# NilFoundation/crypto3-fil-proofs

Hardware: AMD Instinct MI355X
Metric: Groth16 constraints/sec (BLS12-381); MSM G1 Mpoints/s at 2^26 (higher is better)
Workload: dtype u32 limbs (Fq 381-bit / Fr 255-bit Montgomery)

## Files before the change

crypto3-fil-proofs_amd/csrc/ctx.h:

```cpp
#pragma once
#include <hip/hip_runtime.h>
#include <stdint.h>

#include <atomic>
#include <mutex>
#include <stdexcept>
#include <string>
#include <vector>

#include "curve.h"
#include "field.h"
#include "fr29.h"
#include "tune.h"

namespace mi {

struct hip_error : std::runtime_error {
    hipError_t code;
    hip_error(hipError_t c, const std::string &what) : std::runtime_error(what), code(c) {}
};

#define MI_HIP(call)                                                                              \
    do {                                                                                          \
        hipError_t _e = (call);                                                                   \
// ... 139 lines not shown
                keep.push_back(p);
                continue;
            }
            float ms = 0;
            hipEventElapsedTime(&ms, p.a, p.b);
            p.dst->ms += ms;
            p.dst->launches += 1;
            p.dst->units += p.units;
            pool.push_back(p.a);
            pool.push_back(p.b);
        }
        pending.swap(keep);
    }
    ~EventTimer() {
        for (auto &p : pending) {
            hipEventDestroy(p.a);
            hipEventDestroy(p.b);
        }
        for (auto e : pool) hipEventDestroy(e);
    }
};

inline uint64_t next_ctx_uid() {
    static std::atomic<uint64_t> n{1};
    return n.fetch_add(1);
}

struct Ctx {
    const uint64_t uid = next_ctx_uid();
    int device = 0;
    hipStream_t stream = nullptr;
    std::recursive_mutex mu;
    NttTables tw;
    DevBuf scratch[34];
    Stats stats;
    EventTimer timer;
    PinnedBuf pin;
    int64_t inject_oom = 0;
    Ctx *aux = nullptr;
    hipStream_t aux_streams[2] = {nullptr, nullptr};
    hipStream_t plan_stream = nullptr;
    hipEvent_t plan_ev[2] = {nullptr, nullptr};
};

Ctx &ctx_aux(Ctx &c);
void ctx_aux_free(Ctx &c);

struct ScopedTimer {
    Ctx &c;
    KStat *dst;
    uint64_t units;
    hipEvent_t a;
    ScopedTimer(Ctx &ctx, KStat *s, uint64_t u = 0) : c(ctx), dst(s), units(u) {
        a = c.timer.get();
        MI_HIP(hipEventRecord(a, c.stream));
    }
    ~ScopedTimer() {
        hipEvent_t b = nullptr;
        if (!c.timer.pool.empty()) {
            b = c.timer.pool.back();
            c.timer.pool.pop_back();
        } else if (hipEventCreate(&b) != hipSuccess) {
            return;
        }
        if (hipEventRecord(b, c.stream) != hipSuccess) return;
        c.timer.pending.push_back({a, b, dst, units});
    }
};

void debug_sync(Ctx &c, const char *what);
#define MI_LAUNCHED(ctx, name)          \
    do {                                \
        MI_HIP(hipGetLastError());      \
        ::mi::debug_sync((ctx), (name)); \
    } while (0)

void ntt_init_tables(Ctx &c);
void ntt_free_tables(Ctx &c);
void ntt_dif(Ctx &c, fr_t *d, unsigned log_n, bool inverse);
void ntt_dit(Ctx &c, fr_t *d, unsigned log_n, bool inverse);
void bitrev_permute(Ctx &c, fr_t *d, unsigned log_n);
void ntt_coset_roundtrip(Ctx &c, fr_t *d, unsigned log_n, const fr_t &scale);
bool ntt_coset_qap(Ctx &c, fr_t *a, const fr_t *b, fr_t *cc, unsigned log_n, const fr_t &scale, const fr_t &zinv);
void ntt_dif_coset_epilogue(Ctx &c, fr_t *d, unsigned log_n, bool inverse, bool inverse_gen, const fr_t &scale,
                            bool to_canonical);
void coset_scale_bitrev(Ctx &c, fr_t *d, unsigned log_n, bool inverse_gen, const fr_t *scale_host,
                        bool to_canonical);
void coset_scale_natural(Ctx &c, fr_t *d, unsigned log_n, bool inverse_gen, const fr_t *scale_host);
void scale_all(Ctx &c, fr_t *d, uint64_t n, const fr_t &s);
void fr_to_mont_inplace(Ctx &c, fr_t *d, uint64_t n);
void fr_from_mont_inplace(Ctx &c, fr_t *d, uint64_t n);

constexpr unsigned MSM_PLAN_MAXW = 16;
struct MsmPlan {
    uint64_t n = 0;
    uint64_t nreal = 0;
    unsigned cb = 0, nwin = 0;
    uint32_t nbk = 0, nb = 0, L0 = 0, maxcnt = 0, total = 0;
    uint64_t entries = 0;
    bool glv = false;
    const uint32_t *vals_s = nullptr, *off = nullptr, *cnt = nullptr, *coff = nullptr, *ccnt = nullptr,
                   *chunk_bucket = nullptr, *order = nullptr;
    uint32_t m = 0, l1_total = 0, L1 = 16;
    uint32_t level_total[16] = {};
    uint32_t *mlist = nullptr, *qcnt = nullptr, *qoff = nullptr;
    uint32_t wn[MSM_PLAN_MAXW] = {};
    bool marked = false;
};
bool msm_prepare(Ctx &c, const fr_t *scalars, const uint32_t *idx, uint64_t n, MsmPlan &plan, bool split = false);
bool msm_prepare_g1_shared(Ctx &c, const fr_t *scalars, uint64_t n, MsmPlan &plan);
bool msm_prepare_marked(Ctx &c, const fr_t *scalars, uint64_t n, MsmPlan &plan, bool glv, const uint32_t *amark);
bool msm_derive_plan(Ctx &c, const MsmPlan &src, const uint32_t *rank_bits, uint64_t nreal_dst, uint32_t dst_base,
                     MsmPlan &plan);
void msm_g1_planned(Ctx &c, const MsmPlan &plan, const g1_affine_t *bases, g1_xyzz_t *result_host,
                    const g1_affine_t *bases_hi = nullptr);
void msm_g2_planned(Ctx &c, const MsmPlan &plan, const g2_affine_t *bases, g2_xyzz_t *result_host);
struct WinTable {
    const void *p = nullptr;
    uint64_t stride = 0;
    unsigned c = 0, nwin = 0;
    bool sparse = false;
};
unsigned msm_wt_window_bits(uint64_t n);
void g1_window_table(Ctx &c, const g1_affine_t *bases, uint64_t n, unsigned wbits, g1_affine_t *dst);
void g2_window_table(Ctx &c, const g2_affine_t *bases, uint64_t n, unsigned wbits, g2_affine_t *dst);
void msm_g1(Ctx &c, const g1_affine_t *bases, const fr_t *scalars, const uint32_t *idx, uint64_t n,
            g1_xyzz_t *result_host, const g1_affine_t *bases_hi = nullptr, bool subgroup = false,
            const WinTable *wt = nullptr, uint64_t wt_lo = 0);
bool msm_use_split(uint64_t n);
int msm_glv_mode();
void g1_shift128(Ctx &c, const g1_affine_t *in, uint64_t n, g1_affine_t *out);
void msm_g2(Ctx &c, const g2_affine_t *bases, const fr_t *scalars, const uint32_t *idx, uint64_t n,
            g2_xyzz_t *result_host,
            const WinTable *wt = nullptr, uint64_t wt_lo = 0);
unsigned msm_window_bits(uint64_t n);
unsigned msm_window_bits_for(uint64_t n, unsigned sbits, bool glv = false);

void g1_decode_uncompressed(Ctx &c, const uint8_t *dev_bytes, g1_affine_t *out, uint64_t n, int *bad_dev,
                            bool reject_inf = false);
void g2_decode_uncompressed(Ctx &c, const uint8_t *dev_bytes, g2_affine_t *out, uint64_t n, int *bad_dev,
                            bool reject_inf = false);
void g1_subgroup_check(Ctx &c, const g1_affine_t *pts, uint64_t n, int *bad_dev);
void g2_subgroup_check(Ctx &c, const g2_affine_t *pts, uint64_t n, int *bad_dev);
void fr_count_noncanonical(Ctx &c, const fr_t *d, uint64_t n, int *bad_dev, hipStream_t st);
void g1_encode_uncompressed(Ctx &c, const g1_affine_t *in, uint8_t *dev_out, uint64_t n, unsigned perm_log,
                            uint64_t first = 0);
void g2_encode_uncompressed(Ctx &c, const g2_affine_t *in, uint8_t *dev_out, uint64_t n);
void fr_canonicalize(Ctx &c, fr_t *d, uint64_t n);

}
```

crypto3-fil-proofs_amd/csrc/ntt.hip:

```cpp
#include "ctx.h"
#include "fr29.h"

namespace mi {

namespace {

constexpr unsigned TILE_LOG = 10;
constexpr unsigned TILE = 1u << TILE_LOG;
constexpr unsigned NTT_THREADS = 256;
#ifndef MI_NTT_WAVES
#define MI_NTT_WAVES 0
#endif
#if MI_NTT_WAVES
#define MI_NTT_OCC __attribute__((amdgpu_waves_per_eu(MI_NTT_WAVES)))
#else
#define MI_NTT_OCC
#endif

__device__ __forceinline__ fr_t tw_full(const fr_t *__restrict__ lo, const fr_t *__restrict__ hi, uint32_t e) {
    uint32_t l = e & 0xffffu, h = e >> 16;
    if (l == 0) return hi[h];
    if (h == 0) return lo[l];
    return lo[l] * hi[h];
}
// ... 38 lines not shown
__device__ __forceinline__ fr_t to_fr(const fr29_t &x) { return fr_from_fr29(fr29_sub_if_ge(x, FrDesc::MOD29)); }
__device__ __forceinline__ unsigned ins2(unsigned q, unsigned p0) {
    return (q & ((1u << p0) - 1)) | ((q >> p0) << (p0 + 2));
}
__device__ __forceinline__ unsigned ins1(unsigned q, unsigned p) {
    return (q & ((1u << p) - 1)) | ((q >> p) << (p + 1));
}
__device__ __forceinline__ fr29_t tw_b(const fr29_t *__restrict__ tw, unsigned j, unsigned sh) { return tw[j << sh]; }

template <bool DIF>
__device__ __forceinline__ void ntt_rounds(LdsTile &sh, unsigned b, unsigned Tlog, unsigned tile,
                                           const fr29_t *__restrict__ tw10, unsigned tsh) {
    const unsigned T = 1u << Tlog;
    const unsigned nquad = tile >> 2;
    const unsigned nr4 = b >> 1;
    const bool odd = b & 1;
    const unsigned q = threadIdx.x;
    const unsigned bmask = (1u << b) - 1;
    for (unsigned rr = 0; rr < nr4 + (odd ? 1 : 0); rr++) {
        const unsigned r = DIF ? rr : nr4 + (odd ? 1 : 0) - 1 - rr;
        const unsigned s = 2 * r;
        if (r < nr4) {
            if (q < nquad) {
                const unsigned hs = b - 1 - s;
                const unsigned p0 = Tlog + hs - 1;
                const unsigned base = ins2(q, p0);
                const unsigned o1 = 1u << p0, o2 = 2u << p0;
                const unsigned i1 = (base >> Tlog) & bmask;
                const unsigned h = 1u << hs;
                const unsigned j0 = (i1 & (h - 1)) << s;
                const unsigned j1 = j0 + (1u << (b - 2));
                const unsigned jq = (i1 & ((h >> 1) - 1)) << (s + 1);
                fr29_t x0 = lds_get(sh, base), x1 = lds_get(sh, base + o1);
                fr29_t x2 = lds_get(sh, base + o2), x3 = lds_get(sh, base + o2 + o1);
                if (DIF) {
                    fr29_t a = fr29_add(x0, x2), c = fr29_sub_lazy(x0, x2, R2X29);
                    fr29_t bb = fr29_add(x1, x3), dd = fr29_sub_lazy(x1, x3, R2X29);
                    if (j0) c = fr29_mul(c, tw_b(tw10, j0, tsh));
                    dd = fr29_mul(dd, tw_b(tw10, j1, tsh));
                    x0 = red8(fr29_add(a, bb));
                    x1 = fr29_sub_lazy(a, bb, R4X29);
                    x2 = red8(fr29_add(c, dd));
                    x3 = fr29_sub_lazy(c, dd, R2X29);
                    if (jq) {
                        const fr29_t w = tw_b(tw10, jq, tsh);
                        x1 = fr29_mul(x1, w);
                        x3 = fr29_mul(x3, w);
                    } else {
                        x1 = red8(x1);
                        x3 = red8(x3);
                    }
                } else {
                    if (jq) {
                        const fr29_t w = tw_b(tw10, jq, tsh);
                        x1 = fr29_mul(x1, w);
                        x3 = fr29_mul(x3, w);
                    }
                    fr29_t a = fr29_add(x0, x1), bb = fr29_sub_lazy(x0, x1, R2X29);
                    fr29_t c = fr29_add(x2, x3), dd = fr29_sub_lazy(x2, x3, R2X29);
                    if (j0) c = fr29_mul(c, tw_b(tw10, j0, tsh));
                    dd = fr29_mul(dd, tw_b(tw10, j1, tsh));
                    x0 = red8(fr29_add(a, c));
                    x2 = red8(fr29_sub_lazy(a, c, R4X29));
                    x1 = red8(fr29_add(bb, dd));
                    x3 = red8(fr29_sub_lazy(bb, dd, R2X29));
                }
                lds_put(sh, base, x0);
                lds_put(sh, base + o1, x1);
                lds_put(sh, base + o2, x2);
                lds_put(sh, base + o2 + o1, x3);
            }
        } else {
            for (unsigned u = q; u < (tile >> 1); u += NTT_THREADS) {
                const unsigned base = ins1(u, Tlog);
                const fr29_t x0 = lds_get(sh, base), x1 = lds_get(sh, base + T);
                lds_put(sh, base, red4(fr29_add(x0, x1)));
                lds_put(sh, base + T, red4(fr29_sub_lazy(x0, x1, R2X29)));
            }
        }
        __syncthreads();
    }
}

template <bool DIF, bool FUSED = false>
__global__ void __launch_bounds__(NTT_THREADS) MI_NTT_OCC k_ntt_pass(fr_t *__restrict__ d, unsigned L, unsigned M, unsigned b,
                                                          unsigned Tlog, unsigned Glog, int twiddle,
                                                          const fr29_t *__restrict__ lo,
                                                          const fr29_t *__restrict__ hi,
                                                          const fr29_t *__restrict__ tw10, int epi,
                                                          const fr29_t *__restrict__ glo,
                                                          const fr29_t *__restrict__ ghi, fr_t scale,
                                                          const fr29_t *__restrict__ tw10b = nullptr) {
    __shared__ LdsTile sh;
    const fr29_t *twA = tw10, *twB = tw10b;
    const unsigned tsh = TILE_LOG - b;
    const fr29_t sc29 = fr29_from_fr(scale);
    const unsigned T = 1u << Tlog;
    const unsigned Slog = M - b;
    const uint64_t S = 1ull << Slog;
    const unsigned tile_log = Glog + b + Tlog;
    const unsigned tile = 1u << tile_log;
    uint64_t sub0, i20;
    if (Glog > 0) {
        sub0 = (uint64_t)blockIdx.x << Glog;
        i20 = 0;
    } else {
        uint64_t blocks_per_sub = S >> Tlog;
        sub0 = blockIdx.x / blocks_per_sub;
        i20 = (blockIdx.x % blocks_per_sub) << Tlog;
    }
    const unsigned bmask = (1u << b) - 1;
    for (unsigned e = threadIdx.x; e < tile; e += NTT_THREADS) {
        unsigned t = e & (T - 1), i1 = (e >> Tlog) & bmask, g = e >> (Tlog + b);
        uint64_t gi = ((sub0 + g) << M) + ((uint64_t)i1 << Slog) + i20 + t;
        fr29_t x = f29(d[gi]);
        if (!DIF && twiddle) {
            uint32_t k1 = brev(i1, b);
            uint32_t ex = (uint32_t)(((uint64_t)(i20 + t) * k1) << (32 - M));
            if (ex) x = fr29_mul(x, tw29(lo, hi, ex));
        }
        lds_put(sh, e, x);
    }
    __syncthreads();
    ntt_rounds<DIF>(sh, b, Tlog, tile, twA, tsh);
    if (FUSED) {
        for (unsigned e = threadIdx.x; e < tile; e += NTT_THREADS) {
            unsigned t = e & (T - 1), i1 = (e >> Tlog) & bmask, g = e >> (Tlog + b);
            uint64_t gi = ((sub0 + g) << M) + ((uint64_t)i1 << Slog) + i20 + t;
            fr29_t x = lds_get(sh, e);
            uint32_t ex = brev((uint32_t)gi, L);
            if (ex) x = fr29_mul(x, tw29(glo, ghi, ex));
            lds_put(sh, e, fr29_mul(x, sc29));
        }
        __syncthreads();
        ntt_rounds<false>(sh, b, Tlog, tile, twB, tsh);
    }
    for (unsigned e = threadIdx.x; e < tile; e += NTT_THREADS) {
        unsigned t = e & (T - 1), i1 = (e >> Tlog) & bmask, g = e >> (Tlog + b);
        uint64_t gi = ((sub0 + g) << M) + ((uint64_t)i1 << Slog) + i20 + t;
        fr29_t x = lds_get(sh, e);
        if (DIF && !FUSED && twiddle) {
            uint32_t k1 = brev(i1, b);
            uint32_t ex = (uint32_t)(((uint64_t)(i20 + t) * k1) << (32 - M));
            if (ex) x = fr29_mul(x, tw29(lo, hi, ex));
        }
        if (DIF && !FUSED && epi) {
            uint32_t ex = brev((uint32_t)gi, L);
            if (ex) x = fr29_mul(x, tw29(glo, ghi, ex));
            x = fr29_mul(x, sc29);
            if (epi == 2) {
                d[gi] = fr_from_fr29(fr29_from_mont(x));
                continue;
            }
        }
        d[gi] = to_fr(x);
    }
}

__global__ void __launch_bounds__(NTT_THREADS) MI_NTT_OCC k_ntt_qap(fr_t *__restrict__ ha, const fr_t *__restrict__ bv,
                                                         const fr_t *__restrict__ cv, unsigned L, unsigned b,
                                                         unsigned Tlog, const fr29_t *__restrict__ flo,
                                                         const fr29_t *__restrict__ fhi,
                                                         const fr29_t *__restrict__ ftw10,
                                                         const fr29_t *__restrict__ ilo,
                                                         const fr29_t *__restrict__ ihi,
                                                         const fr29_t *__restrict__ itw10, fr_t zinv) {
    __shared__ LdsTile sh;
    const unsigned tsh = TILE_LOG - b;
    const fr29_t z29 = fr29_from_fr(zinv);
    const unsigned T = 1u << Tlog;
    const unsigned Slog = L - b;
    const unsigned tile = 1u << (b + Tlog);
    const uint64_t i20 = (uint64_t)blockIdx.x << Tlog;
    const unsigned bmask = (1u << b) - 1;
    for (unsigned e = threadIdx.x; e < tile; e += NTT_THREADS) {
        const unsigned t = e & (T - 1), i1 = (e >> Tlog) & bmask;
        const uint64_t gi = ((uint64_t)i1 << Slog) + i20 + t;
        fr29_t x = f29(cv[gi]);
        const uint32_t ex = (uint32_t)(((i20 + t) * brev(i1, b)) << (32 - L));
        if (ex) x = fr29_mul(x, tw29(flo, fhi, ex));
        lds_put(sh, e, x);
    }
    __syncthreads();
    ntt_rounds<false>(sh, b, Tlog, tile, ftw10, tsh);
    for (unsigned e = threadIdx.x; e < tile; e += NTT_THREADS) {
        const unsigned t = e & (T - 1), i1 = (e >> Tlog) & bmask;
        const uint64_t gi = ((uint64_t)i1 << Slog) + i20 + t;
        const fr29_t ab = fr29_mul(f29(ha[gi]), f29(bv[gi]));
        lds_put(sh, e, fr29_mul(fr29_sub_lazy(ab, lds_get(sh, e), R2X29), z29));
    }
    __syncthreads();
    ntt_rounds<true>(sh, b, Tlog, tile, itw10, tsh);
    for (unsigned e = threadIdx.x; e < tile; e += NTT_THREADS) {
        const unsigned t = e & (T - 1), i1 = (e >> Tlog) & bmask;
        const uint64_t gi = ((uint64_t)i1 << Slog) + i20 + t;
        fr29_t x = lds_get(sh, e);
        const uint32_t ex = (uint32_t)(((i20 + t) * brev(i1, b)) << (32 - L));
        if (ex) x = fr29_mul(x, tw29(ilo, ihi, ex));
        ha[gi] = to_fr(x);
    }
}

struct PassPlan {
    unsigned M, b, Tlog, Glog;
    bool twiddle;
    uint64_t blocks;
};

std::vector<PassPlan> plan_passes(unsigned L) {
    std::vector<PassPlan> ps;
    if (L == 0) return ps;
    unsigned inner = L < TILE_LOG ? L : TILE_LOG;
    unsigned rest = L - inner;
    unsigned nouter = (rest + 7) / 8;
    std::vector<unsigned> bits;
    for (unsigned i = 0; i < nouter; i++) bits.push_back(rest / nouter + (i < rest % nouter ? 1 : 0));
    bits.push_back(inner);
    unsigned M = L;
    for (size_t p = 0; p < bits.size(); p++) {
        PassPlan pp;
        pp.M = M;
        pp.b = bits[p];
        unsigned Slog = M - pp.b;
        unsigned room = TILE_LOG - pp.b;
        if (Slog >= room) {
            pp.Tlog = room;
            pp.Glog = 0;
            pp.blocks = (1ull << (L - M)) * ((1ull << Slog) >> pp.Tlog);
        } else {
            pp.Tlog = Slog;
            unsigned g = room - Slog;
            unsigned nsub_log = L - M;
            if (g > nsub_log) g = nsub_log;
            pp.Glog = g;
            pp.blocks = 1ull << (nsub_log - g);
        }
        pp.twiddle = (p + 1 < bits.size());
        ps.push_back(pp);
        M -= pp.b;
    }
    return ps;
}

__global__ void k_bitrev_permute(fr_t *__restrict__ d, unsigned L, uint64_t n) {
    uint64_t i = (uint64_t)blockIdx.x * blockDim.x + threadIdx.x;
    if (i >= n) return;
    uint64_t r = L ? (__builtin_bitreverse64(i) >> (64 - L)) : 0;
    if (i < r) {
        fr_t a = d[i], b = d[r];
        d[i] = b;
        d[r] = a;
    }
}

__global__ void k_coset_scale(fr_t *__restrict__ d, unsigned L, uint64_t n, int bitrev_pos,
                              const fr_t *__restrict__ lo, const fr_t *__restrict__ hi, fr_t scale,
                              int use_scale, int to_canonical) {
    uint64_t i = (uint64_t)blockIdx.x * blockDim.x + threadIdx.x;
    if (i >= n) return;
    uint32_t e = bitrev_pos ? brev((uint32_t)i, L) : (uint32_t)i;
    fr_t x = d[i];
    if (e) x = x * tw_full(lo, hi, e);
    if (use_scale) x = x * scale;
    if (to_canonical) x = from_mont(x);
    d[i] = x;
}

__global__ void k_scale(fr_t *__restrict__ d, uint64_t n, fr_t s) {
    uint64_t i = (uint64_t)blockIdx.x * blockDim.x + threadIdx.x;
    if (i < n) d[i] = d[i] * s;
}
__global__ void k_to_mont(fr_t *__restrict__ d, uint64_t n) {
    uint64_t i = (uint64_t)blockIdx.x * blockDim.x + threadIdx.x;
    if (i < n) d[i] = to_mont(d[i]);
}
__global__ void k_from_mont(fr_t *__restrict__ d, uint64_t n) {
    uint64_t i = (uint64_t)blockIdx.x * blockDim.x + threadIdx.x;
    if (i < n) d[i] = from_mont(d[i]);
}

inline unsigned grid1(uint64_t n) { return (unsigned)((n + 255) / 256); }

void host_table(std::vector<fr_t> &lo, std::vector<fr_t> &hi, const fr_t &w) {
    lo.resize(65536);
    hi.resize(65536);
    lo[0] = fr_t::one();
    for (int i = 1; i < 65536; i++) lo[i] = lo[i - 1] * w;
    fr_t w16 = lo[65535] * w;
    hi[0] = fr_t::one();
    for (int i = 1; i < 65536; i++) hi[i] = hi[i - 1] * w16;
}

fr_t fr_small(uint32_t v) {
    fr_t r = fr_t::zero();
    r.v[0] = v;
    return to_mont(r);
}

}

fr_t fr_root_of_unity_2_32() {
    uint32_t e[7];
    for (int i = 0; i < 7; i++) e[i] = FrDesc::MOD[i + 1];
    return pow_words(fr_small(7), e, 7);
}

void ntt_init_tables(Ctx &c) {
    fr_t w = fr_root_of_unity_2_32();
    fr_t t = w;
    for (int i = 0; i < 31; i++) t = sqr(t);
    if (!(t == -fr_t::one())) throw std::runtime_error("ntt: bad 2^32-th root of unity");
    fr_t wi = inverse(w), g = fr_small(7), gi = inverse(g);
    std::vector<fr_t> lo, hi;
    fr_t **dst[4][2] = {{&c.tw.fw_lo, &c.tw.fw_hi}, {&c.tw.iv_lo, &c.tw.iv_hi}, {&c.tw.g_lo, &c.tw.g_hi},
                        {&c.tw.gi_lo, &c.tw.gi_hi}};
    fr_t bases[4] = {w, wi, g, gi};
    for (int k = 0; k < 4; k++) {
        host_table(lo, hi, bases[k]);
        MI_HIP(hipMalloc(dst[k][0], sizeof(fr_t) * 65536));
        MI_HIP(hipMalloc(dst[k][1], sizeof(fr_t) * 65536));
        MI_HIP(hipMemcpy(*dst[k][0], lo.data(), sizeof(fr_t) * 65536, hipMemcpyHostToDevice));
        MI_HIP(hipMemcpy(*dst[k][1], hi.data(), sizeof(fr_t) * 65536, hipMemcpyHostToDevice));
        {
            std::vector<fr29_t> l29(65536), h29(65536);
            for (int i = 0; i < 65536; i++) l29[i] = fr29_from_fr(lo[i]), h29[i] = fr29_from_fr(hi[i]);
            MI_HIP(hipMalloc(&c.tw.lo29[k], sizeof(fr29_t) * 65536));
            MI_HIP(hipMalloc(&c.tw.hi29[k], sizeof(fr29_t) * 65536));
            MI_HIP(hipMemcpy(c.tw.lo29[k], l29.data(), sizeof(fr29_t) * 65536, hipMemcpyHostToDevice));
            MI_HIP(hipMemcpy(c.tw.hi29[k], h29.data(), sizeof(fr29_t) * 65536, hipMemcpyHostToDevice));
        }
        if (k < 2) {
            std::vector<fr29_t> t10(TILE / 2);
            for (unsigned j = 0; j < TILE / 2; j++) t10[j] = fr29_from_fr(hi[j << (16 - TILE_LOG)]);
            fr29_t **p10 = k == 0 ? &c.tw.fw_1024 : &c.tw.iv_1024;
            MI_HIP(hipMalloc(p10, sizeof(fr29_t) * (TILE / 2)));
            MI_HIP(hipMemcpy(*p10, t10.data(), sizeof(fr29_t) * (TILE / 2), hipMemcpyHostToDevice));
        }
    }
}

void ntt_free_tables(Ctx &c) {
    fr_t *ps[8] = {c.tw.fw_lo, c.tw.fw_hi, c.tw.iv_lo, c.tw.iv_hi, c.tw.g_lo, c.tw.g_hi, c.tw.gi_lo, c.tw.gi_hi};
    for (auto p : ps)
        if (p) hipFree(p);
    for (int k = 0; k < 4; k++) {
        if (c.tw.lo29[k]) hipFree(c.tw.lo29[k]);
        if (c.tw.hi29[k]) hipFree(c.tw.hi29[k]);
    }
    if (c.tw.fw_1024) hipFree(c.tw.fw_1024);
    if (c.tw.iv_1024) hipFree(c.tw.iv_1024);
    c.tw = NttTables();
}

static void ntt_run(Ctx &c, fr_t *d, unsigned L, bool inverse, bool dif, int epi = 0, bool inv_gen = false,
// ... 18 lines not shown
            int e = (i + 1 == plan.size()) ? epi : 0;
            k_ntt_pass<true><<<(unsigned)p.blocks, NTT_THREADS, 0, c.stream>>>(d, L, p.M, p.b, p.Tlog, p.Glog,
                                                                                 p.twiddle, lo, hi, tw10, e, glo,
                                                                                 ghi, scale);
        }
    } else {
        for (int i = (int)plan.size() - 1; i >= 0; i--) {
            auto &p = plan[i];
            k_ntt_pass<false><<<(unsigned)p.blocks, NTT_THREADS, 0, c.stream>>>(d, L, p.M, p.b, p.Tlog, p.Glog,
                                                                                  p.twiddle, lo, hi, tw10, 0, glo,
                                                                                  ghi, scale);
        }
    }
    MI_HIP(hipGetLastError());
}

void ntt_coset_roundtrip(Ctx &c, fr_t *d, unsigned L, const fr_t &scale) {
    if (L > 32) throw std::runtime_error("ntt: domain larger than 2^32");
    if (L == 0) {
        scale_all(c, d, 1, scale);
        return;
    }
    ScopedTimer tm(c, &c.stats.ntt, 1ull << L);
    auto plan = plan_passes(L);
    const size_t last = plan.size() - 1;
    for (size_t i = 0; i < last; i++) {
        auto &p = plan[i];
        k_ntt_pass<true><<<(unsigned)p.blocks, NTT_THREADS, 0, c.stream>>>(d, L, p.M, p.b, p.Tlog, p.Glog, p.twiddle,
                                                                             c.tw.lo29[1], c.tw.hi29[1], c.tw.iv_1024, 0,
                                                                             c.tw.lo29[2], c.tw.hi29[2], scale);
    }
    {
        auto &p = plan[last];
        k_ntt_pass<true, true><<<(unsigned)p.blocks, NTT_THREADS, 0, c.stream>>>(
            d, L, p.M, p.b, p.Tlog, p.Glog, 0, c.tw.lo29[1], c.tw.hi29[1], c.tw.iv_1024, 1, c.tw.lo29[2], c.tw.hi29[2],
            scale, c.tw.fw_1024);
    }
    for (int i = (int)last - 1; i >= 0; i--) {
        auto &p = plan[i];
        k_ntt_pass<false><<<(unsigned)p.blocks, NTT_THREADS, 0, c.stream>>>(d, L, p.M, p.b, p.Tlog, p.Glog, p.twiddle,
                                                                              c.tw.lo29[0], c.tw.hi29[0], c.tw.fw_1024, 0,
                                                                              c.tw.lo29[2], c.tw.hi29[2], scale);
    }
    MI_HIP(hipGetLastError());
}

bool ntt_coset_qap(Ctx &c, fr_t *a, const fr_t *b, fr_t *cc, unsigned L, const fr_t &scale, const fr_t &zinv) {
    if (L > 32) throw std::runtime_error("ntt: domain larger than 2^32");
    auto plan = plan_passes(L);
    if (plan.size() < 2) return false;
    {
        ScopedTimer tm(c, &c.stats.ntt, 1ull << L);
        const size_t last = plan.size() - 1;
        for (size_t i = 0; i < last; i++) {
            auto &p = plan[i];
            k_ntt_pass<true><<<(unsigned)p.blocks, NTT_THREADS, 0, c.stream>>>(cc, L, p.M, p.b, p.Tlog, p.Glog, p.twiddle,
                                                                                 c.tw.lo29[1], c.tw.hi29[1], c.tw.iv_1024,
                                                                                 0, c.tw.lo29[2], c.tw.hi29[2], scale);
        }
        {
            auto &p = plan[last];
            k_ntt_pass<true, true><<<(unsigned)p.blocks, NTT_THREADS, 0, c.stream>>>(
                cc, L, p.M, p.b, p.Tlog, p.Glog, 0, c.tw.lo29[1], c.tw.hi29[1], c.tw.iv_1024, 1, c.tw.lo29[2],
                c.tw.hi29[2], scale, c.tw.fw_1024);
        }
        for (size_t i = last - 1; i >= 1; i--) {
            auto &p = plan[i];
            k_ntt_pass<false><<<(unsigned)p.blocks, NTT_THREADS, 0, c.stream>>>(cc, L, p.M, p.b, p.Tlog, p.Glog,
                                                                                  p.twiddle, c.tw.lo29[0], c.tw.hi29[0],
                                                                                  c.tw.fw_1024, 0, c.tw.lo29[2],
                                                                                  c.tw.hi29[2], scale);
        }
        auto &p0 = plan[0];
        if (p0.M != L || p0.Glog != 0 || !p0.twiddle) throw std::logic_error("ntt: unexpected outer pass shape");
        k_ntt_qap<<<(unsigned)p0.blocks, NTT_THREADS, 0, c.stream>>>(a, b, cc, L, p0.b, p0.Tlog, c.tw.lo29[0],
                                                                     c.tw.hi29[0], c.tw.fw_1024, c.tw.lo29[1],
                                                                     c.tw.hi29[1], c.tw.iv_1024, zinv);
        MI_HIP(hipGetLastError());
    }
    ntt_run(c, a, L, true, true, 2, true, scale, 1);
    return true;
}

void ntt_dif_coset_epilogue(Ctx &c, fr_t *d, unsigned log_n, bool inverse, bool inverse_gen, const fr_t &scale,
                            bool to_canonical) {
    ntt_run(c, d, log_n, inverse, true, to_canonical ? 2 : 1, inverse_gen, scale);
}

void ntt_dif(Ctx &c, fr_t *d, unsigned log_n, bool inverse) { ntt_run(c, d, log_n, inverse, true); }
void ntt_dit(Ctx &c, fr_t *d, unsigned log_n, bool inverse) { ntt_run(c, d, log_n, inverse, false); }

void bitrev_permute(Ctx &c, fr_t *d, unsigned log_n) {
    uint64_t n = 1ull << log_n;
    k_bitrev_permute<<<grid1(n), 256, 0, c.stream>>>(d, log_n, n);
    MI_HIP(hipGetLastError());
}

void coset_scale_bitrev(Ctx &c, fr_t *d, unsigned log_n, bool inverse_gen, const fr_t *scale_host,
                        bool to_canonical) {
    uint64_t n = 1ull << log_n;
    k_coset_scale<<<grid1(n), 256, 0, c.stream>>>(d, log_n, n, 1, inverse_gen ? c.tw.gi_lo : c.tw.g_lo,
                                                  inverse_gen ? c.tw.gi_hi : c.tw.g_hi,
                                                  scale_host ? *scale_host : fr_t::one(), scale_host != nullptr,
                                                  to_canonical);
    MI_HIP(hipGetLastError());
}

void coset_scale_natural(Ctx &c, fr_t *d, unsigned log_n, bool inverse_gen, const fr_t *scale_host) {
    uint64_t n = 1ull << log_n;
    k_coset_scale<<<grid1(n), 256, 0, c.stream>>>(d, log_n, n, 0, inverse_gen ? c.tw.gi_lo : c.tw.g_lo,
                                                  inverse_gen ? c.tw.gi_hi : c.tw.g_hi,
                                                  scale_host ? *scale_host : fr_t::one(), scale_host != nullptr, 0);
    MI_HIP(hipGetLastError());
}

void scale_all(Ctx &c, fr_t *d, uint64_t n, const fr_t &s) {
    k_scale<<<grid1(n), 256, 0, c.stream>>>(d, n, s);
    MI_HIP(hipGetLastError());
}
void fr_to_mont_inplace(Ctx &c, fr_t *d, uint64_t n) {
    if (!n) return;
    k_to_mont<<<grid1(n), 256, 0, c.stream>>>(d, n);
    MI_HIP(hipGetLastError());
}
void fr_from_mont_inplace(Ctx &c, fr_t *d, uint64_t n) {
    if (!n) return;
    k_from_mont<<<grid1(n), 256, 0, c.stream>>>(d, n);
    MI_HIP(hipGetLastError());
}

}
```

crypto3-fil-proofs_amd/csrc/prover.hip:

```cpp
#include <hipcub/hipcub.hpp>

#include <string.h>

#include <atomic>
#include <exception>
#include <cstring>
#include <future>
#include <mutex>
#include <string>
#include <thread>
#include <unordered_map>

#include "prover.h"
#include "hostfield.h"
#include <future>

namespace mi {

namespace {

inline unsigned grid1(uint64_t n) { return (unsigned)((n + 255) / 256); }

fr_t fr_small_mont(uint32_t v) {
    fr_t r = fr_t::zero();
// ... 1159 lines not shown
        S->n_l = circ.n_aux;
        if (circ.n_aux) {
            k_lc_scalars<<<grid1(circ.n_aux), 256, 0, st>>>(S->at, S->bt, S->ct, circ.n_in, circ.n_aux, alpha, beta,
                                                            delta_inv, ks);
            S->l = dalloc<g1_affine_t>(circ.n_aux);
            fixed_base_affine<fq_t>(c, t1, ks, circ.n_aux, S->l);
        }
        {
            k_lc_scalars<<<grid1(circ.n_in), 256, 0, st>>>(S->at, S->bt, S->ct, 0, circ.n_in, alpha, beta, gamma_inv,
                                                           ks);
            std::vector<fr_t> ick(circ.n_in);
            MI_HIP(hipMemcpyAsync(ick.data(), ks, 32 * circ.n_in, hipMemcpyDeviceToHost, st));
            MI_HIP(hipStreamSynchronize(st));
            S->n_ic = circ.n_in;
            S->ic.resize(circ.n_in);
            for (uint64_t i = 0; i < circ.n_in; i++) S->ic[i] = host_mul_affine(g1, ick[i]);
        }
        S->n_a = circ.n_a;
        k_gather_canon<<<grid1(circ.n_a), 256, 0, st>>>(S->at, circ.idx_a, circ.n_a, ks);
        S->a = dalloc<g1_affine_t>(circ.n_a);
        fixed_base_affine<fq_t>(c, t1, ks, circ.n_a, S->a);
        S->n_b = circ.n_b;
        if (circ.n_b) {
            k_gather_canon<<<grid1(circ.n_b), 256, 0, st>>>(S->bt, circ.idx_b, circ.n_b, ks);
            S->b_g1 = dalloc<g1_affine_t>(circ.n_b);
            S->b_g2 = dalloc<g2_affine_t>(circ.n_b);
            fixed_base_affine<fq_t>(c, t1, ks, circ.n_b, S->b_g1);
            fixed_base_affine<fq2_t>(c, t2, ks, circ.n_b, S->b_g2);
        }
        MI_HIP(hipStreamSynchronize(st));
        ks_t.reset();
        pw_t.reset();
        t1_t.reset();
        t2_t.reset();
        for (auto &b : c.scratch) b.release();
        for (Ctx *x = c.aux; x; x = x->aux)
            for (auto &b : x->scratch) b.release();
        S->alpha_g1 = host_mul_affine(g1, toxic_canonical[1]);
        S->beta_g1 = host_mul_affine(g1, toxic_canonical[2]);
        S->delta_g1 = host_mul_affine(g1, toxic_canonical[4]);
        S->beta_g2 = host_mul_affine(g2, toxic_canonical[2]);
        S->gamma_g2 = host_mul_affine(g2, toxic_canonical[3]);
        S->delta_g2 = host_mul_affine(g2, toxic_canonical[4]);
        build_hi_tables(c, *S, circ.idx_a, circ.n_in, circ.n_aux);
    } catch (...) {
        (void)hipStreamSynchronize(st);
        delete S;
        throw;
    }
    srs_publish(S);
    return S;
}
}

Srs *srs_generate(Ctx &c, const Circuit &circ, const fr_t toxic_canonical[5]) {
    try {
        return srs_generate_once(c, circ, toxic_canonical);
    } catch (const hip_error &e) {
        if (e.code != hipErrorOutOfMemory) throw;
        c.stats.oom_retries += 1;
        c.stats.oom_freed_bytes += release_for_retry(c, nullptr, nullptr);
        return srs_generate_once(c, circ, toxic_canonical);
    }
}

namespace {
fr_t *compute_h(Ctx &c, const Circuit &circ, const fr_t *z_dev) {
    hipStream_t st = c.stream;
    const uint64_t d = circ.d, nv = circ.n_in + circ.n_aux;
    const unsigned L = circ.log_d;
    fr_t *zm = c.scratch[20].as<fr_t>(nv + 3 * d);
    fr_t *a = zm + nv, *b = a + d, *cc = b + d;
    k_copy_to_mont<<<grid1(nv), 256, 0, st>>>(z_dev, zm, nv);
    eval_witness_map(c, circ, zm, a, b, cc);
    fr_t dd = fr_t::zero();
    dd.v[0] = (uint32_t)d;
    dd.v[1] = (uint32_t)(d >> 32);
    fr_t dinv = inverse(to_mont(dd));
    fr_t g = fr_small_mont(7);
    fr_t zinv = inverse(pow_u64(g, d) - fr_t::one());
    const bool qap_fused = tune::get(tune::QAP_FUSED, 1) != 0;
    ntt_coset_roundtrip(c, a, L, dinv);
    ntt_coset_roundtrip(c, b, L, dinv);
    if (!qap_fused || !ntt_coset_qap(c, a, b, cc, L, dinv, zinv)) {
        ntt_coset_roundtrip(c, cc, L, dinv);
        k_qap_divide<<<grid1(d), 256, 0, st>>>(a, b, cc, d, zinv);
        ntt_dif_coset_epilogue(c, a, L, true, true, dinv, true);
    }
    return a;
}

ProofSums groth16_sums_once(Ctx &c, const Srs &srs, const Circuit &circ, const fr_t *z_dev, const SumRanges &rg,
                            bool inject_oom, const fr_t *h_in) {
    std::shared_lock<std::shared_mutex> in_use(srs.use_mu);
    if (srs.d != circ.d || srs.n_l != circ.n_aux || srs.n_a != circ.n_a || srs.n_b != circ.n_b)
        throw std::invalid_argument("SRS does not match circuit");
    const uint64_t totals[4] = {circ.d - 1, circ.n_aux, circ.n_a, circ.n_b};
    for (int q = 0; q < 4; q++)
        if (rg.lo[q] > totals[q] || rg.cnt[q] > totals[q] - rg.lo[q])
            throw std::invalid_argument("MSM range past the end of its query");
    hipStream_t st = c.stream;
    const uint64_t d = circ.d, nv = circ.n_in + circ.n_aux;
    const unsigned L = circ.log_d;
    const bool need_h = rg.cnt[0] > 0;
    ProofSums out;
    g1_xyzz_t &H = out.H, &Lq = out.L, &As = out.A, &B1 = out.B1;
    g2_xyzz_t &B2 = out.B2;
    out.premul = rg.premul_r && rg.premul_s;
    auto premul_b1 = [&] {
        if (out.premul) out.rB1 = host::xyzz_mul(B1, rg.premul_r->v, 8);
    };
    {
    ScopedTimer whole(c, &c.stats.prove, circ.n);
    {
        const bool one_lane = tune::get(tune::PROVE_LANES, 2) == 1;
        const int64_t wl = tune::get(tune::PROVE_WIDE_LOG, 21);
        const unsigned wide_log = wl >= 0 && wl < 64 ? (unsigned)wl : 21u;
        const bool wide = !one_lane && L <= wide_log;
        const unsigned nlanes = wide ? 3 : 1;
        Ctx *lane_ctx[3] = {one_lane ? &c : &ctx_aux(c), nullptr, nullptr};
        for (unsigned k = 1; k < nlanes; k++) lane_ctx[k] = &ctx_aux(*lane_ctx[k - 1]);
        hipEvent_t ready = c.timer.get(), done[3] = {nullptr, nullptr, nullptr};
        MI_HIP(hipEventRecord(ready, st));
        for (unsigned k = 0; k < nlanes; k++) {
            done[k] = lane_ctx[k]->timer.get();
            MI_HIP(hipStreamWaitEvent(lane_ctx[k]->stream, ready, 0));
        }
        std::exception_ptr err[3];
        const int64_t b1t = tune::get(tune::PROVE_B1_LANE, 2);
        const unsigned b1_lane = wide ? (b1t < 0 || b1t > 2 ? 2u : (unsigned)b1t) : 0u;
        auto run_b = [&](Ctx &x) {
            const uint64_t lo = rg.lo[3], cnt = rg.cnt[3];
            WinTable wt2 = srs.wt_of(4);
            wt2.sparse = true;
            if (b1_lane != 0 && wt2.p) {
                msm_g2(x, srs.b_g2 + lo, z_dev, circ.idx_b + lo, cnt, &B2, &wt2, lo);
                return;
            }
            MsmPlan pb;
            msm_prepare(x, z_dev, circ.idx_b + lo, cnt, pb);
            if (b1_lane == 0) {
                msm_g1_planned(x, pb, srs.b_g1 + lo, &B1);
                premul_b1();
            }
            msm_g2_planned(x, pb, srs.b_g2 + lo, &B2);
        };
        auto run_b1 = [&](Ctx &x) {
            const uint64_t lo = rg.lo[3], cnt = rg.cnt[3];
            WinTable wt = srs.wt_of(3);
            wt.sparse = true;
            msm_g1(x, srs.b_g1 + lo, z_dev, circ.idx_b + lo, cnt, &B1, nullptr, srs.in_subgroup, &wt, lo);
            premul_b1();
        };
        auto run_l = [&](Ctx &x) {
            const uint64_t l_lo = rg.lo[1], l_cnt = rg.cnt[1];
            WinTable wt = srs.wt_of(1);
            wt.sparse = true;
            msm_g1(x, srs.l + l_lo, z_dev + circ.n_in + l_lo, nullptr, l_cnt, &Lq, srs.l_hi ? srs.l_hi + l_lo : nullptr,
                   srs.in_subgroup, &wt, l_lo);
        };
        auto run_a = [&](Ctx &x) {
            const uint64_t a_lo = rg.lo[2], a_cnt = rg.cnt[2];
            WinTable wt = srs.wt_of(2);
            wt.sparse = true;
            msm_g1(x, srs.a + a_lo, z_dev, circ.idx_a + a_lo, a_cnt, &As, srs.a_hi ? srs.a_hi + a_lo : nullptr,
                   srs.in_subgroup, &wt, a_lo);
            if (out.premul) out.sA = host::xyzz_mul(As, rg.premul_s->v, 8);
// ... 415 lines not shown
```

crypto3-fil-proofs_amd/csrc/tune.h:

```cpp
#pragma once
#include <atomic>
#include <climits>
#include <cstdint>
#include <cstring>

namespace mi::tune {

enum Knob : int {
    MSM_C = 0,
    MSM_SPLIT,
    MSM_SPLIT_MIN,
    MSM_GLV,
    MSM_WT,
    MSM_WT_C,
    MSM_WT_MAX_LOG,
    MSM_L0,
    MSM_L1,
    MSM_SORT,
    MSM_BITSUM,
    MSM_SEGA_LOG,
    MSM_SEGB_LOG,
    MSM_BS_SEG_LOG,
    MSM_BS_G0,
    G2_L2,
    G2_AFF_K,
    QAP_FUSED,
    PROVE_LANES,
    PROVE_WIDE_LOG,
    PROVE_B1_LANE,
    AUX_ORDER,
    LANE_PRIO,
    WIT_POS_LANES,
    SDR_PREFETCH,
    POSEIDON_PAIR,
    TREE_BATCH,
    DEBUG_SYNC,
    PLAN_PRIO,
    A_FROM_L,
    NKNOBS
};

constexpr int64_t UNSET = INT64_MIN;

inline constexpr const char *kNames[NKNOBS] = {
    "msm_c",          "msm_split",      "msm_split_min",  "msm_glv",       "msm_wt",         "msm_wt_c",
    "msm_wt_max_log", "msm_l0",         "msm_l1",         "msm_sort",      "msm_bitsum",     "msm_sega_log",
    "msm_segb_log",   "msm_bs_seg_log", "msm_bs_g0",      "g2_l2",         "g2_aff_k",       "qap_fused",
    "prove_lanes",    "prove_wide_log", "prove_b1_lane",  "aux_order",     "lane_prio",      "wit_pos_lanes",
    "sdr_prefetch",   "poseidon_pair",  "tree_batch",     "debug_sync",    "plan_prio",
    "a_from_l"};

inline std::atomic<int64_t> g_knobs[NKNOBS] = {};
inline std::atomic<bool> g_init{false};

inline void reset() {
    for (int k = 0; k < NKNOBS; k++) g_knobs[k].store(UNSET, std::memory_order_relaxed);
    g_init.store(true, std::memory_order_release);
}

inline int find(const char *name) {
    if (!name) return -1;
    for (int k = 0; k < NKNOBS; k++)
        if (strcmp(kNames[k], name) == 0) return k;
    return -1;
}

inline int64_t get(Knob k, int64_t dflt) {
    if (!g_init.load(std::memory_order_acquire)) return dflt;
    const int64_t v = g_knobs[k].load(std::memory_order_relaxed);
    return v == UNSET ? dflt : v;
}

inline bool is_set(Knob k) { return get(k, UNSET) != UNSET; }

inline void set(Knob k, int64_t v) {
    static const bool once = (reset(), true);
    (void)once;
    g_knobs[k].store(v, std::memory_order_relaxed);
}

}
```

Before: 148.6 million.

## Compute QAP quotient via linearity, dropping the C coset NTT roundtrip

Adds a default-on QAP path that exploits linearity. C is inverse-transformed directly instead of taking a full coset roundtrip. The pointwise A*B product then goes through a single inverse coset NTT, and C is subtracted and scaled by zinv*dinv in the final pass. In the fused variant the A*B multiply is folded into the first NTT pass and the coset twiddle, subtraction and scaling into the last pass. This removes roughly two full-size NTTs and extra memory sweeps, but relies on the algebraic equivalence holding exactly, including Montgomery and canonical form handling.

```diff
diff --git a/crypto3-fil-proofs_amd/csrc/ctx.h b/crypto3-fil-proofs_amd/csrc/ctx.h
--- a/crypto3-fil-proofs_amd/csrc/ctx.h
+++ b/crypto3-fil-proofs_amd/csrc/ctx.h
@@ -245,6 +245,8 @@
 void bitrev_permute(Ctx &c, fr_t *d, unsigned log_n);
 void ntt_coset_roundtrip(Ctx &c, fr_t *d, unsigned log_n, const fr_t &scale);
 bool ntt_coset_qap(Ctx &c, fr_t *a, const fr_t *b, fr_t *cc, unsigned log_n, const fr_t &scale, const fr_t &zinv);
+void ntt_qap_linear(Ctx &c, fr_t *a, const fr_t *b, fr_t *cc, unsigned log_n, const fr_t &dinv, const fr_t &zinv,
+                    bool fused);
 void ntt_dif_coset_epilogue(Ctx &c, fr_t *d, unsigned log_n, bool inverse, bool inverse_gen, const fr_t &scale,
                             bool to_canonical);
 void coset_scale_bitrev(Ctx &c, fr_t *d, unsigned log_n, bool inverse_gen, const fr_t *scale_host,
diff --git a/crypto3-fil-proofs_amd/csrc/ntt.hip b/crypto3-fil-proofs_amd/csrc/ntt.hip
--- a/crypto3-fil-proofs_amd/csrc/ntt.hip
+++ b/crypto3-fil-proofs_amd/csrc/ntt.hip
@@ -144,7 +144,7 @@
     }
 }
 
-template <bool DIF, bool FUSED = false>
+template <bool DIF, bool FUSED = false, int QAP = 0>
 __global__ void __launch_bounds__(NTT_THREADS) MI_NTT_OCC k_ntt_pass(fr_t *__restrict__ d, unsigned L, unsigned M, unsigned b,
                                                           unsigned Tlog, unsigned Glog, int twiddle,
                                                           const fr29_t *__restrict__ lo,
@@ -152,7 +152,8 @@
                                                           const fr29_t *__restrict__ tw10, int epi,
                                                           const fr29_t *__restrict__ glo,
                                                           const fr29_t *__restrict__ ghi, fr_t scale,
-                                                          const fr29_t *__restrict__ tw10b = nullptr) {
+                                                          const fr29_t *__restrict__ tw10b = nullptr,
+                                                          const fr_t *__restrict__ aux = nullptr) {
     __shared__ LdsTile sh;
     const fr29_t *twA = tw10, *twB = tw10b;
     const unsigned tsh = TILE_LOG - b;
@@ -176,6 +177,7 @@
         unsigned t = e & (T - 1), i1 = (e >> Tlog) & bmask, g = e >> (Tlog + b);
         uint64_t gi = ((sub0 + g) << M) + ((uint64_t)i1 << Slog) + i20 + t;
         fr29_t x = f29(d[gi]);
+        if (QAP & 1) x = fr29_mul(x, f29(aux[gi]));
         if (!DIF && twiddle) {
             uint32_t k1 = brev(i1, b);
             uint32_t ex = (uint32_t)(((uint64_t)(i20 + t) * k1) << (32 - M));
@@ -205,6 +207,12 @@
             uint32_t k1 = brev(i1, b);
             uint32_t ex = (uint32_t)(((uint64_t)(i20 + t) * k1) << (32 - M));
             if (ex) x = fr29_mul(x, tw29(lo, hi, ex));
+        }
+        if (QAP & 2) {
+            uint32_t ex = brev((uint32_t)gi, L);
+            if (ex) x = fr29_mul(x, tw29(glo, ghi, ex));
+            d[gi] = to_fr(fr29_mul(fr29_sub_lazy(x, f29(aux[gi]), FrDesc::MOD29), sc29));
+            continue;
         }
         if (DIF && !FUSED && epi) {
             uint32_t ex = brev((uint32_t)gi, L);
@@ -332,6 +340,19 @@
     uint64_t i = (uint64_t)blockIdx.x * blockDim.x + threadIdx.x;
     if (i < n) d[i] = d[i] * s;
 }
+__global__ void k_mul_into(fr_t *__restrict__ a, const fr_t *__restrict__ b, uint64_t n) {
+    uint64_t i = (uint64_t)blockIdx.x * blockDim.x + threadIdx.x;
+    if (i < n) a[i] = a[i] * b[i];
+}
+__global__ void k_qap_linear_epilogue(fr_t *__restrict__ a, const fr_t *__restrict__ c, unsigned L, uint64_t n,
+                                      const fr_t *__restrict__ lo, const fr_t *__restrict__ hi, fr_t s) {
+    uint64_t i = (uint64_t)blockIdx.x * blockDim.x + threadIdx.x;
+    if (i >= n) return;
+    uint32_t e = brev((uint32_t)i, L);
+    fr_t x = a[i];
+    if (e) x = x * tw_full(lo, hi, e);
+    a[i] = from_mont((x - c[i]) * s);
+}
 __global__ void k_to_mont(fr_t *__restrict__ d, uint64_t n) {
     uint64_t i = (uint64_t)blockIdx.x * blockDim.x + threadIdx.x;
     if (i < n) d[i] = to_mont(d[i]);
@@ -516,6 +537,43 @@
     return true;
 }
 
+void ntt_qap_linear(Ctx &c, fr_t *a, const fr_t *b, fr_t *cc, unsigned L, const fr_t &dinv, const fr_t &zinv,
+                    bool fused) {
+    if (L > 32) throw std::runtime_error("ntt: domain larger than 2^32");
+    const uint64_t n = 1ull << L;
+    const fr_t s = zinv * dinv;
+    ntt_run(c, cc, L, true, true);
+    auto plan = plan_passes(L);
+    if (!fused || plan.size() < 2) {
+        k_mul_into<<<grid1(n), 256, 0, c.stream>>>(a, b, n);
+        MI_HIP(hipGetLastError());
+        ntt_run(c, a, L, true, true);
+        k_qap_linear_epilogue<<<grid1(n), 256, 0, c.stream>>>(a, cc, L, n, c.tw.gi_lo, c.tw.gi_hi, s);
+        MI_HIP(hipGetLastError());
+        return;
+    }
+    ScopedTimer tm(c, &c.stats.ntt, n);
+    const fr_t s_canon = from_mont(s);
+    const fr29_t *lo = c.tw.lo29[1], *hi = c.tw.hi29[1], *glo = c.tw.lo29[3], *ghi = c.tw.hi29[3];
+    const size_t last = plan.size() - 1;
+    {
+        auto &p = plan[0];
+        k_ntt_pass<true, false, 1><<<(unsigned)p.blocks, NTT_THREADS, 0, c.stream>>>(
+            a, L, p.M, p.b, p.Tlog, p.Glog, p.twiddle, lo, hi, c.tw.iv_1024, 0, glo, ghi, s_canon, nullptr, b);
+    }
+    for (size_t i = 1; i < last; i++) {
+        auto &p = plan[i];
+        k_ntt_pass<true><<<(unsigned)p.blocks, NTT_THREADS, 0, c.stream>>>(a, L, p.M, p.b, p.Tlog, p.Glog, p.twiddle,
+                                                                             lo, hi, c.tw.iv_1024, 0, glo, ghi, s_canon);
+    }
+    {
+        auto &p = plan[last];
+        k_ntt_pass<true, false, 2><<<(unsigned)p.blocks, NTT_THREADS, 0, c.stream>>>(
+            a, L, p.M, p.b, p.Tlog, p.Glog, p.twiddle, lo, hi, c.tw.iv_1024, 0, glo, ghi, s_canon, nullptr, cc);
+    }
+    MI_HIP(hipGetLastError());
+}
+
 void ntt_dif_coset_epilogue(Ctx &c, fr_t *d, unsigned log_n, bool inverse, bool inverse_gen, const fr_t &scale,
                             bool to_canonical) {
     ntt_run(c, d, log_n, inverse, true, to_canonical ? 2 : 1, inverse_gen, scale);
diff --git a/crypto3-fil-proofs_amd/csrc/prover.hip b/crypto3-fil-proofs_amd/csrc/prover.hip
--- a/crypto3-fil-proofs_amd/csrc/prover.hip
+++ b/crypto3-fil-proofs_amd/csrc/prover.hip
@@ -1265,7 +1265,9 @@
     const bool qap_fused = tune::get(tune::QAP_FUSED, 1) != 0;
     ntt_coset_roundtrip(c, a, L, dinv);
     ntt_coset_roundtrip(c, b, L, dinv);
-    if (!qap_fused || !ntt_coset_qap(c, a, b, cc, L, dinv, zinv)) {
+    if (tune::get(tune::QAP_LINEAR, 1) != 0) {
+        ntt_qap_linear(c, a, b, cc, L, dinv, zinv, qap_fused);
+    } else if (!qap_fused || !ntt_coset_qap(c, a, b, cc, L, dinv, zinv)) {
         ntt_coset_roundtrip(c, cc, L, dinv);
         k_qap_divide<<<grid1(d), 256, 0, st>>>(a, b, cc, d, zinv);
         ntt_dif_coset_epilogue(c, a, L, true, true, dinv, true);
diff --git a/crypto3-fil-proofs_amd/csrc/tune.h b/crypto3-fil-proofs_amd/csrc/tune.h
--- a/crypto3-fil-proofs_amd/csrc/tune.h
+++ b/crypto3-fil-proofs_amd/csrc/tune.h
@@ -37,6 +37,7 @@
     DEBUG_SYNC,
     PLAN_PRIO,
     A_FROM_L,
+    QAP_LINEAR,
     NKNOBS
 };
 
@@ -48,7 +49,7 @@
     "msm_segb_log",   "msm_bs_seg_log", "msm_bs_g0",      "g2_l2",         "g2_aff_k",       "qap_fused",
     "prove_lanes",    "prove_wide_log", "prove_b1_lane",  "aux_order",     "lane_prio",      "wit_pos_lanes",
     "sdr_prefetch",   "poseidon_pair",  "tree_batch",     "debug_sync",    "plan_prio",
-    "a_from_l"};
+    "a_from_l",       "qap_linear"};
 
 inline std::atomic<int64_t> g_knobs[NKNOBS] = {};
 inline std::atomic<bool> g_init{false};
```

Result: faster. 152.5 million, median of 6 (+2.6%).
